# hila-chefer/Transformer-Explainability

Hardware: NVIDIA H100
Metric: explanations_per_sec (higher is better)
Workload: dtype f32

## Files before the change

transformer_explainability_b200/csrc/te_api.cu:

```cuda
#include <stdlib.h>
#include <string.h>
#include <atomic>
#include <string>

#include "../../include/te_b200.h"
#include "te_engine_util.h"
#include "te_kernels.h"
#include "te_rollout.h"
#include "te_zplus.h"
#include "te_gemm_tc.h"

static thread_local std::string g_last_error;
void te_set_last_error(const char* msg) { g_last_error = msg ? msg : ""; }

static std::atomic<long long> g_launches{0};
void te_count_launch() { g_launches.fetch_add(1, std::memory_order_relaxed); }
extern "C" long long te_kernel_launch_count(void) { return g_launches.load(); }

extern "C" const char* te_last_error(void) { return g_last_error.c_str(); }
extern "C" int te_version(void) { return 101; }

#define ST(s) reinterpret_cast<cudaStream_t>(s)
#define REQ(c, msg) do { if (!(c)) { te_set_last_error(msg); return TE_ERR_ARG; } } while (0)

// ... 214 lines not shown
void te_engine_set_cls_rows(int on) { g_cls_rows = on ? 1 : 0; }
static int g_gelu_split = -1;
bool te_engine_gelu_split() {
    if (g_gelu_split < 0) {
        const char* e = getenv("TE_B200_GELU_SPLIT");
        g_gelu_split = (e && e[0] == '0') ? 0 : 1;
    }
    return g_gelu_split != 0;
}
void te_engine_set_gelu_split(int on) { g_gelu_split = on ? 1 : 0; }

extern "C" int te_set_option(const char* name, int value) {
    REQ(name != nullptr, "te_set_option: null name");
    if (strcmp(name, "cls_row_top_block") == 0) { te_engine_set_cls_rows(value); return TE_OK; }
    if (strcmp(name, "gelu_split_fused") == 0) { te_engine_set_gelu_split(value); return TE_OK; }
    te_set_last_error("te_set_option: unknown option");
    return TE_ERR_ARG;
}

extern "C" int te_relevance_heatmap(const float* maps, int batch, int grid, int scale, float* out, void* stream) {
    REQ(maps && out && batch > 0 && grid > 0 && scale > 0, "te_relevance_heatmap: bad argument");
    return te_launch_relevance_heatmap(maps, out, batch, grid, scale, ST(stream));
}

extern "C" int te_head_reduce(const float* a, const float* g, const float* head_w, int batch, int heads, int n, int ld,
                              int mode, float* out, void* stream) {
    REQ(a && out && batch > 0 && heads > 0 && n > 0 && ld >= n && mode >= 0 && mode <= 2, "te_head_reduce: bad argument");
    return te_launch_head_reduce(a, g, head_w, out, batch, heads, n, ld, mode, ST(stream));
}
extern "C" int te_head_region_mean(const float* g, int batch, int heads, int n, int ld, int r0, int r1, int c0, int c1,
// ... 78 lines not shown
```

transformer_explainability_b200/csrc/te_gemm_tc.h:

```cpp
#pragma once
#include <cuda_bf16.h>
#include <type_traits>

#include "te_common.cuh"
#include "te_zplus.h"

bool te_tc_zplus_supported(long long rows, int in_features, int out_features, long long ldx);

template <class F>
struct TeDerived {
    template <class T> using P = std::conditional_t<std::is_const<F>::value, const T*, T*>;
    F *wp, *wn, *wpt, *wnt;
    F *wh, *wl, *wth, *wtl;
    F* wabs;
    P<__nv_bfloat16> bf_wpt, bf_wnt;
    F* gap;
    P<__nv_bfloat16> bf_wabs;
    P<__half> h_w, l_w;
    F* s_w;
    P<__half> h_wt;
    F* s_wt;
    P<__half> h_wpt, h_wnt;
    F *s_wpt, *s_wnt;
    static constexpr long long floats(int in_features, int out_features) { return 16LL * in_features * out_features; }
// ... 66 lines not shown
```

transformer_explainability_b200/csrc/te_tc_wgmma.cu:

```cuda
#include <cuda.h>
#include <cuda_bf16.h>
#include <cuda_fp16.h>
#include <cuda_runtime.h>
#include <string.h>
#include <algorithm>
#include <string>
#include <type_traits>
#include <utility>

#include "te_gemm_tc.h"
#include "te_wgmma.cuh"

namespace {

constexpr int BM = 128, NTHREADS = 256;

__device__ __forceinline__ uint32_t smem_u32(const void* p) { return (uint32_t)__cvta_generic_to_shared(p); }
__device__ __forceinline__ void fence_proxy_async() { asm volatile("fence.proxy.async.shared::cta;" ::: "memory"); }
__device__ __forceinline__ void wg_fence() { asm volatile("wgmma.fence.sync.aligned;" ::: "memory"); }
__device__ __forceinline__ void wg_commit() { asm volatile("wgmma.commit_group.sync.aligned;" ::: "memory"); }
__device__ __forceinline__ void wg_wait0() { asm volatile("wgmma.wait_group.sync.aligned 0;" ::: "memory"); }
__device__ __forceinline__ void wg_wait1() { asm volatile("wgmma.wait_group.sync.aligned 1;" ::: "memory"); }

__device__ __forceinline__ void mbar_init(uint32_t bar, uint32_t count) {
// ... 75 lines not shown
struct Stage {
    static constexpr int NTA = PRODS::NTA, NTB = PRODS::NTB;
    static constexpr int BYTES = NTA * TILE128 + NTB * BN * 128 + LAND;
    __host__ __device__ static constexpr uint32_t a(int i) { return (uint32_t)i * TILE128; }
    __host__ __device__ static constexpr uint32_t b(int j) { return (uint32_t)(NTA * TILE128 + j * BN * 128); }
    __host__ __device__ static constexpr uint32_t land() { return (uint32_t)(NTA * TILE128 + NTB * BN * 128); }
};

enum { OP_TF32 = 0, OP_BF16 = 1, OP_F16 = 2 };
template <int FMT, int NR>
__device__ __forceinline__ void wgmma_fmt(float (&d)[NR], uint64_t a, uint64_t b, uint32_t scale_d) {
    if constexpr (FMT == OP_TF32) wgmma_tf32(d, a, b, scale_d);
    else if constexpr (FMT == OP_BF16) wgmma_bf16(d, a, b, scale_d);
    else wgmma_f16(d, a, b, scale_d);
}
template <int FMT, class... T, size_t... I, int NA, int NR, int TA, int TB>
__device__ __forceinline__ void issue_kstep(Prods<T...>, std::index_sequence<I...>, float (&acc)[NA][NR], const uint64_t (&a)[TA],
                                            const uint64_t (&b)[TB], uint64_t q, uint32_t sd) {
    (wgmma_fmt<FMT>(acc[T::acc], a[T::a] + q, b[T::b] + q, Prods<T...>::first(I) ? sd : 1u), ...);
}
template <class P, int NA, int NR>
__device__ __forceinline__ void issue(uint32_t st, int wg, float (&acc)[NA][NR], uint32_t sd) {
    using L = typename P::L;
    uint64_t a[L::NTA], b[L::NTB];
#pragma unroll
    for (int i = 0; i < L::NTA; ++i) a[i] = sdesc(st + L::a(i) + (uint32_t)wg * 64u * 128u);
#pragma unroll
    for (int j = 0; j < L::NTB; ++j) b[j] = sdesc(st + L::b(j));
#pragma unroll
    for (int k = 0; k < 4; ++k)
        issue_kstep<P::FMT>(typename P::PRODS{}, std::make_index_sequence<P::PRODS::N>{}, acc, a, b, (uint64_t)(2 * k),
                            (k == 0) ? sd : 1u);
}

template <class F>
__device__ __forceinline__ void for_k32(int rows, const float* __restrict__ base, long long ld, long long row0, long long nrows,
                                        int k0, int K, int tid, F f) {
    for (int idx = tid; idx < rows * 8; idx += NTHREADS) {
        const int r = idx >> 3, c = idx & 7;
        const long long gr = row0 + r;
        const int k = k0 + 4 * c;
        float4 v = make_float4(0.f, 0.f, 0.f, 0.f);
        if (gr < nrows) {
            const float* src = base + gr * ld + k;
            if (k + 3 < K) v = *reinterpret_cast<const float4*>(src);
            else {
                if (k < K) v.x = src[0];
// ... 97 lines not shown
    const int tid = threadIdx.x, wg = tid >> 7;
    const int m0 = (col_fast ? blockIdx.y : blockIdx.x) * BM, n0 = (col_fast ? blockIdx.x : blockIdx.y) * P::BN;
    const int z = blockIdx.z;
    float acc[NA][NR];
    float tot[NT][NTR];
    zero(acc);
    zero(tot);

    const int kb = p.kblocks();
    p.load(smem, 0, m0, n0, z, tid);
    fence_proxy_async();
    __syncthreads();
    for (int it = 0; it < kb; ++it) {
        const bool fresh = P::CHUNK ? (it % P::CHUNK == 0) : (it == 0);
        wg_fence();
        issue<P>(smem_u32(smem + (it & 1) * STAGE), wg, acc, fresh ? 0u : 1u);
        wg_commit();
        if (it + 1 < kb) p.load(smem + ((it + 1) & 1) * STAGE, it + 1, m0, n0, z, tid);
        wg_wait0();
        if constexpr (P::CHUNK > 0)
            if ((it + 1) % P::CHUNK == 0 || it + 1 == kb) fold(p, acc, tot, m0, it / P::CHUNK, z, tid);
        fence_proxy_async();
        __syncthreads();
    }
    if constexpr (P::CHUNK > 0) p.epilogue(tot, m0, n0, z, tid, nullptr);
    else p.epilogue(acc, m0, n0, z, tid, nullptr);
}

template <class P>
__device__ __forceinline__ void tma_tiles(const P& p, const TmaArgs& ta, uint8_t* smem) {
    using L = typename P::L;
    constexpr int NR = P::BN / 2;
    constexpr int NA = P::PRODS::NACC;
    constexpr int STAGE = L::BYTES, EPI = epi_bytes<P>(), S = tma_stages(STAGE, EPI);
    constexpr int NT = P::CHUNK ? NA : 1, NTR = P::CHUNK ? NR : 1;
    static_assert(S >= 2, "a TMA problem needs two stages");
    __shared__ __align__(8) uint64_t bars[2 * S + 2];
    const int tid = threadIdx.x, wg = tid >> 7;
    const uint32_t full0 = smem_u32(bars), empty0 = full0 + 8u * S, st0 = smem_u32(smem);
    const uint32_t efull = full0 + 16u * S, eempty = efull + 8u, ebuf = st0 + (uint32_t)S * STAGE;
    if (tid == 0) {
        for (int s = 0; s < S; ++s) {
            mbar_init(full0 + 8u * s, 1);
            mbar_init(empty0 + 8u * s, 8);
        }
        mbar_init(efull, 1);
// ... 34 lines not shown
                                         m0, efull);
                        ephase ^= 1u;
                    }
                }
            }
        }
        return;
    }

    setmaxnreg_inc<232>();
    float acc[NA][NR];
    float tot[NT][NTR];
    auto release = [&](int s) {
        if ((tid & 31) == 0) mbar_arrive(empty0 + 8u * s);
    };
    auto consume = [&](uint32_t sd) {
        mbar_wait(full0 + 8u * stage, phase);
        if constexpr (P::FIX != FIX_NONE) {
            p.fix(smem + (uint32_t)stage * STAGE, wg, tid);
            fence_proxy_async();
            if constexpr (P::FIX == FIX_A) bar_named(1 + wg, 128);
            else bar_named(3, 256);
        }
        wg_fence();
        issue<P>(st0 + (uint32_t)stage * STAGE, wg, acc, sd);
        wg_commit();
    };
    auto next = [&] {
        if (++stage == S) { stage = 0; phase ^= 1u; }
    };
    constexpr int CH = P::CHUNK;
    uint32_t ephase = 0;
    for (int t = blockIdx.x; t < ntiles; t += gridDim.x) {
        int m0, n0, z;
        decode(t, m0, n0, z);
        zero(acc);
        zero(tot);
        for (int k0 = 0; k0 < kb; k0 += CH ? CH : kb) {
            const int k1 = CH ? min(k0 + CH, kb) : kb;
            consume(0u);
            for (int it = k0 + 1; it < k1; ++it) {
                const int prev = stage;
                next();
                consume(1u);
                wg_wait1();
                release(prev);
            }
            wg_wait0();
            release(stage);
            next();
            if constexpr (CH > 0) fold(p, acc, tot, m0, k0 / CH, z, tid);
        }
        if constexpr (EPI > 0) mbar_wait(efull, ephase);
        if constexpr (P::CHUNK > 0) p.epilogue(tot, m0, n0, z, tid, smem + (uint32_t)S * STAGE);
        else p.epilogue(acc, m0, n0, z, tid, smem + (uint32_t)S * STAGE);
        if constexpr (EPI > 0) {
            __syncwarp();
            if ((tid & 31) == 0) mbar_arrive(eempty);
            ephase ^= 1u;
        }
    }
}

template <class P>
__global__ void __launch_bounds__(P::TMA ? NTHREADS_TMA : NTHREADS, 1)
    wg_kernel(const P p, const __grid_constant__ TmaArgs ta, int col_fast) {
    extern __shared__ uint8_t smem_raw[];
    uint8_t* smem = smem_raw + ((1024u - (smem_u32(smem_raw) & 1023u)) & 1023u);
    if constexpr (P::TMA) tma_tiles(p, ta, smem);
    else reg_tile(p, smem, col_fast);
}

struct NoScale {
    __device__ __forceinline__ float chunk_scale(int, int, int) const { return 1.f; }
};

struct TmaTile {
    const void* base;
    long long rows, cols, ld;
    int box_rows;
    long long count = 0, cstride = 0;
};
template <class P>
__device__ __forceinline__ void produce_tiles(const TmaArgs& ta, uint32_t st, uint32_t bar, int it, int m0, int n0) {
// ... 256 lines not shown
    const void* b; const void* b_lo;
    const float* rs; const float* cs;
    LinOut o;
};
static_assert(sizeof(LinArgs) <= 128, "LinArgs: keep the kernel parameter within 128 bytes");
template <int EPI, int FORM>
struct LinProb : LinArgs {
    static constexpr bool F16 = FORM == LIN_F16X3 || FORM == LIN_F16, SPLIT = FORM == LIN_3XTF32 || FORM == LIN_F16X3;
    static constexpr int BN = FORM == LIN_TF32 && EPI == TE_TC_EPI_STORE ? 256 : 128;
    static constexpr int CHUNK = F16 ? 2 : SPLIT ? 4 : 0, FMT = F16 ? OP_F16 : OP_TF32;
    using PRODS = std::conditional_t<SPLIT, Split3, One>;
    using L = Stage<PRODS, BN>;
    static constexpr bool COL_FAST = true;
    static constexpr bool TMA = FORM != LIN_3XTF32;
    static constexpr int FIX = FORM == LIN_TF32 ? FIX_A : FIX_NONE;
    static constexpr int EPI_MAPS = TMA && EPI == TE_TC_EPI_GELU_BWD ? 1 : 0;
    __device__ int kblocks() const { return K / (F16 ? 64 : 32); }
    __device__ float chunk_scale(int row, int ch, int) const {
        if constexpr (F16) return row < o.M ? rs[(long long)row * rs_ld + ch] : 1.f;
        else return 1.f;
    }
    __device__ void fix(uint8_t* st, int wg, int tid) const {
        map_rows(st + L::a(0), 64 * wg, 64, tid & 127, 128, [](float4 v) { return tf32x4(v); });
    }
    TE_PRODUCE_TILES(LinProb)
    TmaTile tile(int i) const {
        if (i < L::NTA) return TmaTile{i == 0 ? a : a_lo, o.M, K, F16 ? K : lda, BM};
        if (i < NMAPS) return TmaTile{i == L::NTA ? b : b_lo, o.N, K, K, BN};
        return TmaTile{o.E, o.M, o.N, o.lde, BM};
    }
// ... 31 lines not shown
    }
    __device__ float2 efrag(const uint8_t* eb, int tid, int j, int row, int col) const {
        if constexpr (EPI_MAPS > 0) return epi_f2(eb, frag_row(tid, j), frag_col(tid, j));
        else return *reinterpret_cast<const float2*>(o.E + (long long)row * o.lde + col);
    }
};

enum { AT_STORE = 0, AT_MUL = 1, AT_SD = 2, AT_SOFTMAX = 3, AT_RESID = 4 };
template <int EPI, bool SP, int BN_>
struct NnProb : NoScale {
    static constexpr int BN = BN_, CHUNK = 0, FMT = OP_TF32;
    using PRODS = std::conditional_t<SP, One, Split3>;
    using L = Stage<PRODS, BN>;
    static constexpr bool TMA = true;
    static constexpr int FIX = FIX_AB, EPI_MAPS = 0;
    int N, H, dh, ld_out, batch;
    const float* a; long long lda; const float* b; long long ldb;
    const float* E; float* out; float alpha;
    __device__ int kblocks() const { return dh / 32; }
    static constexpr int NMAPS = 2;
    TmaTile tile(int i) const {
        return i == 0 ? TmaTile{a, (long long)batch * N, H * dh, lda, BM} : TmaTile{b, (long long)batch * N, H * dh, ldb, BN};
    }
    __device__ void produce(const TmaArgs& ta, uint32_t st, uint32_t bar, int kb, int m0, int n0, int bh) const {
        const int s = bh / H, k = (bh % H) * dh + kb * 32;
        mbar_expect_tx(bar, TILE128 + BN * 128);
        tma_load(st + L::a(0), &ta.map[0], k, s * N + m0, bar);
        tma_load(st + L::b(0), &ta.map[1], k, s * N + n0, bar);
    }
    __device__ void fix(uint8_t* st, int wg, int tid) const {
        fix_tf32<SP>(st + L::a(0), st + L::a(1), 64 * wg, 64, tid & 127, 128);
        fix_tf32<SP>(st + L::b(0), st + L::b(1), 0, BN, tid, 256);
    }
    __device__ void epilogue(float (&acc)[1][BN / 2], int m0, int n0, int bh, int tid, const uint8_t*) const {
        const int ncols = (N + 3) & ~3;
        if constexpr (EPI == AT_SOFTMAX) {
            float mx[2] = {-INFINITY, -INFINITY};
#pragma unroll
            for (int j = 0; j < BN / 2; ++j)
                if (n0 + frag_col(tid, j) < N) mx[(j >> 1) & 1] = fmaxf(mx[(j >> 1) & 1], alpha * acc[0][j]);
            float sum[2] = {0.f, 0.f}, m2[2];
#pragma unroll
            for (int h = 0; h < 2; ++h) {
                mx[h] = fmaxf(mx[h], __shfl_xor_sync(0xffffffffu, mx[h], 1));
                mx[h] = fmaxf(mx[h], __shfl_xor_sync(0xffffffffu, mx[h], 2));
                m2[h] = -mx[h] * 1.4426950408889634f;
            }
            const float a2 = alpha * 1.4426950408889634f;
// ... 40 lines not shown
            }
            *reinterpret_cast<float2*>(out + off) = make_float2(v[0], v[1]);
        }
        }
    }
};

template <int AMN, int EPI, bool SP, int BN_>
struct NkProb : NoScale {
    static constexpr int BN = BN_, CHUNK = SP ? 0 : 4, FMT = OP_TF32;
    using PRODS = std::conditional_t<SP, One, Split3>;
    static constexpr int LAND_A = AMN ? BM * 128 : 0, LAND_X = BN * 128;
    using L = Stage<PRODS, BN, LAND_A + LAND_X>;
    static constexpr bool TMA = true;
    static constexpr int FIX = FIX_AB, EPI_MAPS = 0;
    int N, H, NP, ld_out, n_out, n_pad, a_shared, batch;
    const float* map; const float* X; long long ldx;
    const float* rowscale; const float* E; float* out; float alpha;
    __device__ int kblocks() const { return (N + 31) / 32; }
    static constexpr int NMAPS = 2;
    TmaTile tile(int i) const {
        if (i == 0) return TmaTile{map, N, N, NP, AMN ? 32 : BM, (long long)batch * (a_shared ? 1 : H), (long long)N * NP};
        return TmaTile{X, N, n_pad, ldx, 32, batch, (long long)N * ldx};
    }
    __device__ void produce(const TmaArgs& ta, uint32_t st, uint32_t bar, int kb, int m0, int, int bh) const {
        const int s = bh / H, h = bh % H, za = a_shared ? s : bh;
        mbar_expect_tx(bar, (AMN ? LAND_A : TILE128) + LAND_X);
        if (AMN == 0) tma_load3(st + L::a(0), &ta.map[0], kb * 32, m0, za, bar);
#pragma unroll
        for (int j = 0; j < LAND_A / 4096; ++j) tma_load3(st + L::land() + j * 4096, &ta.map[0], m0 + 32 * j, kb * 32, za, bar);
#pragma unroll
        for (int j = 0; j < LAND_X / 4096; ++j)
            tma_load3(st + L::land() + LAND_A + j * 4096, &ta.map[1], h * BN + 32 * j, kb * 32, s, bar);
    }
    __device__ void fix(uint8_t* st, int wg, int tid) const {
        if (AMN) transpose_rows(st + L::land(), 64 * wg, 64, tid & 127, 128, put_tf32<SP>(st + L::a(0), st + L::a(1)));
        else fix_tf32<SP>(st + L::a(0), st + L::a(1), 64 * wg, 64, tid & 127, 128);
        transpose_rows(st + L::land() + LAND_A, 0, BN, tid, 256, put_tf32<SP>(st + L::b(0), st + L::b(1)));
    }
    __device__ void epilogue(float (&acc)[1][BN / 2], int m0, int, int bh, int tid, const uint8_t*) const {
        const int s = bh / H, h = bh % H;
        float2 ef[BN / 4];
#pragma unroll
        for (int j = 0; j < BN / 2; j += 2) {
            const int m = m0 + frag_row(tid, j), gcol = h * BN + frag_col(tid, j);
            ef[j / 2] = (EPI != AT_STORE && m < N && gcol < n_pad)
                            ? *reinterpret_cast<const float2*>(E + ((long long)s * N + m) * ld_out + gcol) : make_float2(0.f, 0.f);
        }
#pragma unroll
        for (int j = 0; j < BN / 2; j += 2) {
            const int m = m0 + frag_row(tid, j), gcol = h * BN + frag_col(tid, j);
            if (m >= N || gcol >= n_pad) continue;
// ... 39 lines not shown
    return fn;
}
bool encode_tile(CUtensorMap* map, const TmaTile& t, int esize) {
    const EncodeTiled fn = encode_tiled();
    const int rank = t.count > 0 ? 3 : 2;
    if (!fn || ((uintptr_t)t.base & 15u) || (t.ld * esize) % 16 != 0 || (t.cstride * esize) % 16 != 0 || t.rows < 1 || t.cols < 1)
        return false;
    const cuuint64_t dims[3] = {(cuuint64_t)t.cols, (cuuint64_t)t.rows, (cuuint64_t)t.count};
    const cuuint64_t strides[2] = {(cuuint64_t)(t.ld * esize), (cuuint64_t)(t.cstride * esize)};
    const cuuint32_t box[3] = {(cuuint32_t)(128 / esize), (cuuint32_t)t.box_rows, 1}, estr[3] = {1, 1, 1};
    return fn(map, esize == 4 ? CU_TENSOR_MAP_DATA_TYPE_FLOAT32 : CU_TENSOR_MAP_DATA_TYPE_UINT16, rank, const_cast<void*>(t.base),
              dims, strides, box, estr, CU_TENSOR_MAP_INTERLEAVE_NONE, CU_TENSOR_MAP_SWIZZLE_128B,
              CU_TENSOR_MAP_L2_PROMOTION_L2_256B, CU_TENSOR_MAP_FLOAT_OOB_FILL_NONE) == CUDA_SUCCESS;
}

template <class P>
int launch(const P& p, dim3 grid, cudaStream_t st) {
    TmaArgs ta;
    memset(&ta, 0, sizeof(ta));
    int col_fast = 0, threads = NTHREADS, smem = 2 * P::L::BYTES + 1024;
    if constexpr (P::TMA) {
        constexpr int ESIZE = P::FMT == OP_TF32 ? 4 : 2;
        static_assert(P::NMAPS + P::EPI_MAPS <= TMA_MAPS, "TmaArgs holds TMA_MAPS tensor maps");
        for (int i = 0; i < P::NMAPS + P::EPI_MAPS; ++i)
            if (!encode_tile(&ta.map[i], p.tile(i), i < P::NMAPS ? ESIZE : 4)) {
                te_set_last_error("te_tc: cannot encode a TMA tensor map (16-byte-aligned base and strides required)");
                return TE_ERR_ARG;
            }
        const long long tiles = (long long)grid.x * grid.y * grid.z;
        if (tiles > INT32_MAX) { te_set_last_error("te_tc: grid too large for one launch"); return TE_ERR_ARG; }
        ta.mtiles = (int)grid.x;
        ta.ntiles = (int)grid.y;
        ta.nz = (int)grid.z;
        grid = dim3((unsigned)std::min<long long>(tiles, sm_count()));
        threads = NTHREADS_TMA;
        smem = tma_stages(P::L::BYTES, epi_bytes<P>()) * P::L::BYTES + epi_bytes<P>() + 1024;
    } else {
        col_fast = P::COL_FAST && grid.x <= 65535;
        if (col_fast) grid = dim3(grid.y, grid.x, grid.z);
    }
    static unsigned long long done = 0;
    int dev = 0;
    if (cudaGetDevice(&dev) != cudaSuccess) { te_set_last_error("te_tc: cudaGetDevice failed"); return TE_ERR_CUDA; }
    if (!(done & (1ull << (dev & 63)))) {
        if (cudaFuncSetAttribute(wg_kernel<P>, cudaFuncAttributeMaxDynamicSharedMemorySize, smem) != cudaSuccess) {
            te_set_last_error("te_tc: cannot raise dynamic shared memory");
            return TE_ERR_CUDA;
        }
        done |= 1ull << (dev & 63);
    }
    if (grid.y > 65535 || grid.z > 65535) { te_set_last_error("te_tc: grid too large for one launch"); return TE_ERR_ARG; }
    wg_kernel<P><<<grid, threads, smem, st>>>(p, ta, col_fast);
    TE_CUDA_CHECK_LAUNCH();
    return TE_OK;
}
inline unsigned mtiles(long long M) { return (unsigned)((M + BM - 1) / BM); }

__global__ void prepare_weights_kernel(const float* __restrict__ w, float* __restrict__ d, int out_f, int in_f) {
    const TeDerived<float> dv(d, in_f, out_f);
    __shared__ float tile[32][33];
    const int bx = blockIdx.x * 32, by = blockIdx.y * 32;
    for (int i = threadIdx.y; i < 32; i += blockDim.y) {
        const int o = by + i, c = bx + threadIdx.x;
        float v = 0.f;
        if (o < out_f && c < in_f) {
            const long long idx = (long long)o * in_f + c;
            v = w[idx];
            dv.wp[idx] = to_tf32(fmaxf(v, 0.f));
            dv.wn[idx] = to_tf32(fminf(v, 0.f));
// ... 119 lines not shown
template <bool SINGLE, bool BF, int OUT>
int zs(const float* x, long long ldx, const void* xabs, const void* wa, const void* wb, const float* r, long long ldr,
       const float* y, long long ldy, const float* bias, void* out, float* hs, long long rows, int in_features, int out_features,
       cudaStream_t st, float s_scale, bool inh) {
    ZsProb<SINGLE, BF, OUT> p;
    p.M = (int)rows; p.N = out_features; p.K = in_features;
    p.x = x; p.ldx = ldx; p.xabs = xabs; p.wa = wa; p.wb = wb;
    p.r = r; p.ldr = ldr; p.y = y; p.ldy = ldy; p.bias = bias;
    p.out = out; p.ldo = out_features; p.hs = hs;
    p.sscale = s_scale; p.zsign = inh ? -1.f : 1.f;
    return launch(p, dim3(mtiles(p.M), p.N / 128), st);
}

}

long long te_tc_derived_floats(int in_features, int out_features) { return TeDerived<float>::floats(in_features, out_features); }

int te_tc_prepare_weights(const float* w, float* derived, int in_features, int out_features, cudaStream_t st) {
    dim3 grid((in_features + 31) / 32, (out_features + 31) / 32), block(32, 8);
    prepare_weights_kernel<<<grid, block, 0, st>>>(w, derived, out_features, in_features);
    TE_CUDA_CHECK_LAUNCH();
    const TeDerived<float> dv(derived, in_features, out_features);
    if (in_features % 8 == 0 && in_features >= 8 && a16(w))
        TE_TRY(te_tc_rowsplit_f16(w, in_features, out_features, in_features, dv.h_w, dv.l_w, dv.s_w, st));
    if (out_features % 8 == 0 && in_features >= 2) {
        TE_TRY(te_tc_rowsplit_f16(dv.wth, out_features, in_features, out_features, dv.h_wt, nullptr, dv.s_wt, st));
        TE_TRY(te_tc_rowsplit_f16(dv.wpt, out_features, in_features, out_features, dv.h_wpt, nullptr, dv.s_wpt, st));
        TE_TRY(te_tc_rowsplit_f16(dv.wnt, out_features, in_features, out_features, dv.h_wnt, nullptr, dv.s_wnt, st));
    }
    return TE_OK;
// ... 305 lines not shown
```

transformer_explainability_b200/csrc/te_wgmma.cuh:

```cuda
#pragma once
#include <stdint.h>

__device__ __forceinline__ void wgmma_tf32(float (&d)[32], uint64_t a, uint64_t b, uint32_t scale_d) {
    asm volatile(
        "{\n.reg .pred p;\nsetp.ne.b32 p, %34, 0;\n"
        "wgmma.mma_async.sync.aligned.m64n64k8.f32.tf32.tf32 {%0, %1, %2, %3, %4, %5, %6, %7, %8, %9, %10, %11, %12, %13, %14, %15, %16, %17, %18, %19, %20, %21, %22, %23, %24, %25, %26, %27, %28, %29, %30, %31}, %32, %33, p, 1, 1;\n}\n"
        : "+f"(d[0]), "+f"(d[1]), "+f"(d[2]), "+f"(d[3]), "+f"(d[4]), "+f"(d[5]), "+f"(d[6]), "+f"(d[7]), "+f"(d[8]), "+f"(d[9]), "+f"(d[10]), "+f"(d[11]), "+f"(d[12]), "+f"(d[13]), "+f"(d[14]), "+f"(d[15]), "+f"(d[16]), "+f"(d[17]), "+f"(d[18]), "+f"(d[19]), "+f"(d[20]), "+f"(d[21]), "+f"(d[22]), "+f"(d[23]), "+f"(d[24]), "+f"(d[25]), "+f"(d[26]), "+f"(d[27]), "+f"(d[28]), "+f"(d[29]), "+f"(d[30]), "+f"(d[31])
        : "l"(a), "l"(b), "r"(scale_d));
}
__device__ __forceinline__ void wgmma_tf32(float (&d)[64], uint64_t a, uint64_t b, uint32_t scale_d) {
    asm volatile(
        "{\n.reg .pred p;\nsetp.ne.b32 p, %66, 0;\n"
        "wgmma.mma_async.sync.aligned.m64n128k8.f32.tf32.tf32 {%0, %1, %2, %3, %4, %5, %6, %7, %8, %9, %10, %11, %12, %13, %14, %15, %16, %17, %18, %19, %20, %21, %22, %23, %24, %25, %26, %27, %28, %29, %30, %31, %32, %33, %34, %35, %36, %37, %38, %39, %40, %41, %42, %43, %44, %45, %46, %47, %48, %49, %50, %51, %52, %53, %54, %55, %56, %57, %58, %59, %60, %61, %62, %63}, %64, %65, p, 1, 1;\n}\n"
        : "+f"(d[0]), "+f"(d[1]), "+f"(d[2]), "+f"(d[3]), "+f"(d[4]), "+f"(d[5]), "+f"(d[6]), "+f"(d[7]), "+f"(d[8]), "+f"(d[9]), "+f"(d[10]), "+f"(d[11]), "+f"(d[12]), "+f"(d[13]), "+f"(d[14]), "+f"(d[15]), "+f"(d[16]), "+f"(d[17]), "+f"(d[18]), "+f"(d[19]), "+f"(d[20]), "+f"(d[21]), "+f"(d[22]), "+f"(d[23]), "+f"(d[24]), "+f"(d[25]), "+f"(d[26]), "+f"(d[27]), "+f"(d[28]), "+f"(d[29]), "+f"(d[30]), "+f"(d[31]), "+f"(d[32]), "+f"(d[33]), "+f"(d[34]), "+f"(d[35]), "+f"(d[36]), "+f"(d[37]), "+f"(d[38]), "+f"(d[39]), "+f"(d[40]), "+f"(d[41]), "+f"(d[42]), "+f"(d[43]), "+f"(d[44]), "+f"(d[45]), "+f"(d[46]), "+f"(d[47]), "+f"(d[48]), "+f"(d[49]), "+f"(d[50]), "+f"(d[51]), "+f"(d[52]), "+f"(d[53]), "+f"(d[54]), "+f"(d[55]), "+f"(d[56]), "+f"(d[57]), "+f"(d[58]), "+f"(d[59]), "+f"(d[60]), "+f"(d[61]), "+f"(d[62]), "+f"(d[63])
        : "l"(a), "l"(b), "r"(scale_d));
}
__device__ __forceinline__ void wgmma_tf32(float (&d)[128], uint64_t a, uint64_t b, uint32_t scale_d) {
    asm volatile(
        "{\n.reg .pred p;\nsetp.ne.b32 p, %130, 0;\n"
        "wgmma.mma_async.sync.aligned.m64n256k8.f32.tf32.tf32 {%0, %1, %2, %3, %4, %5, %6, %7, %8, %9, %10, %11, %12, %13, %14, %15, %16, %17, %18, %19, %20, %21, %22, %23, %24, %25, %26, %27, %28, %29, %30, %31, %32, %33, %34, %35, %36, %37, %38, %39, %40, %41, %42, %43, %44, %45, %46, %47, %48, %49, %50, %51, %52, %53, %54, %55, %56, %57, %58, %59, %60, %61, %62, %63, %64, %65, %66, %67, %68, %69, %70, %71, %72, %73, %74, %75, %76, %77, %78, %79, %80, %81, %82, %83, %84, %85, %86, %87, %88, %89, %90, %91, %92, %93, %94, %95, %96, %97, %98, %99, %100, %101, %102, %103, %104, %105, %106, %107, %108, %109, %110, %111, %112, %113, %114, %115, %116, %117, %118, %119, %120, %121, %122, %123, %124, %125, %126, %127}, %128, %129, p, 1, 1;\n}\n"
        : "+f"(d[0]), "+f"(d[1]), "+f"(d[2]), "+f"(d[3]), "+f"(d[4]), "+f"(d[5]), "+f"(d[6]), "+f"(d[7]), "+f"(d[8]), "+f"(d[9]), "+f"(d[10]), "+f"(d[11]), "+f"(d[12]), "+f"(d[13]), "+f"(d[14]), "+f"(d[15]), "+f"(d[16]), "+f"(d[17]), "+f"(d[18]), "+f"(d[19]), "+f"(d[20]), "+f"(d[21]), "+f"(d[22]), "+f"(d[23]), "+f"(d[24]), "+f"(d[25]), "+f"(d[26]), "+f"(d[27]), "+f"(d[28]), "+f"(d[29]), "+f"(d[30]), "+f"(d[31]), "+f"(d[32]), "+f"(d[33]), "+f"(d[34]), "+f"(d[35]), "+f"(d[36]), "+f"(d[37]), "+f"(d[38]), "+f"(d[39]), "+f"(d[40]), "+f"(d[41]), "+f"(d[42]), "+f"(d[43]), "+f"(d[44]), "+f"(d[45]), "+f"(d[46]), "+f"(d[47]), "+f"(d[48]), "+f"(d[49]), "+f"(d[50]), "+f"(d[51]), "+f"(d[52]), "+f"(d[53]), "+f"(d[54]), "+f"(d[55]), "+f"(d[56]), "+f"(d[57]), "+f"(d[58]), "+f"(d[59]), "+f"(d[60]), "+f"(d[61]), "+f"(d[62]), "+f"(d[63]), "+f"(d[64]), "+f"(d[65]), "+f"(d[66]), "+f"(d[67]), "+f"(d[68]), "+f"(d[69]), "+f"(d[70]), "+f"(d[71]), "+f"(d[72]), "+f"(d[73]), "+f"(d[74]), "+f"(d[75]), "+f"(d[76]), "+f"(d[77]), "+f"(d[78]), "+f"(d[79]), "+f"(d[80]), "+f"(d[81]), "+f"(d[82]), "+f"(d[83]), "+f"(d[84]), "+f"(d[85]), "+f"(d[86]), "+f"(d[87]), "+f"(d[88]), "+f"(d[89]), "+f"(d[90]), "+f"(d[91]), "+f"(d[92]), "+f"(d[93]), "+f"(d[94]), "+f"(d[95]), "+f"(d[96]), "+f"(d[97]), "+f"(d[98]), "+f"(d[99]), "+f"(d[100]), "+f"(d[101]), "+f"(d[102]), "+f"(d[103]), "+f"(d[104]), "+f"(d[105]), "+f"(d[106]), "+f"(d[107]), "+f"(d[108]), "+f"(d[109]), "+f"(d[110]), "+f"(d[111]), "+f"(d[112]), "+f"(d[113]), "+f"(d[114]), "+f"(d[115]), "+f"(d[116]), "+f"(d[117]), "+f"(d[118]), "+f"(d[119]), "+f"(d[120]), "+f"(d[121]), "+f"(d[122]), "+f"(d[123]), "+f"(d[124]), "+f"(d[125]), "+f"(d[126]), "+f"(d[127])
        : "l"(a), "l"(b), "r"(scale_d));
}
__device__ __forceinline__ void wgmma_f16(float (&d)[32], uint64_t a, uint64_t b, uint32_t scale_d) {
// ... 12 lines not shown
}
__device__ __forceinline__ void wgmma_bf16(float (&d)[32], uint64_t a, uint64_t b, uint32_t scale_d) {
    asm volatile(
        "{\n.reg .pred p;\nsetp.ne.b32 p, %34, 0;\n"
        "wgmma.mma_async.sync.aligned.m64n64k16.f32.bf16.bf16 {%0, %1, %2, %3, %4, %5, %6, %7, %8, %9, %10, %11, %12, %13, %14, %15, %16, %17, %18, %19, %20, %21, %22, %23, %24, %25, %26, %27, %28, %29, %30, %31}, %32, %33, p, 1, 1, 0, 0;\n}\n"
        : "+f"(d[0]), "+f"(d[1]), "+f"(d[2]), "+f"(d[3]), "+f"(d[4]), "+f"(d[5]), "+f"(d[6]), "+f"(d[7]), "+f"(d[8]), "+f"(d[9]), "+f"(d[10]), "+f"(d[11]), "+f"(d[12]), "+f"(d[13]), "+f"(d[14]), "+f"(d[15]), "+f"(d[16]), "+f"(d[17]), "+f"(d[18]), "+f"(d[19]), "+f"(d[20]), "+f"(d[21]), "+f"(d[22]), "+f"(d[23]), "+f"(d[24]), "+f"(d[25]), "+f"(d[26]), "+f"(d[27]), "+f"(d[28]), "+f"(d[29]), "+f"(d[30]), "+f"(d[31])
        : "l"(a), "l"(b), "r"(scale_d));
}
__device__ __forceinline__ void wgmma_bf16(float (&d)[64], uint64_t a, uint64_t b, uint32_t scale_d) {
    asm volatile(
        "{\n.reg .pred p;\nsetp.ne.b32 p, %66, 0;\n"
        "wgmma.mma_async.sync.aligned.m64n128k16.f32.bf16.bf16 {%0, %1, %2, %3, %4, %5, %6, %7, %8, %9, %10, %11, %12, %13, %14, %15, %16, %17, %18, %19, %20, %21, %22, %23, %24, %25, %26, %27, %28, %29, %30, %31, %32, %33, %34, %35, %36, %37, %38, %39, %40, %41, %42, %43, %44, %45, %46, %47, %48, %49, %50, %51, %52, %53, %54, %55, %56, %57, %58, %59, %60, %61, %62, %63}, %64, %65, p, 1, 1, 0, 0;\n}\n"
        : "+f"(d[0]), "+f"(d[1]), "+f"(d[2]), "+f"(d[3]), "+f"(d[4]), "+f"(d[5]), "+f"(d[6]), "+f"(d[7]), "+f"(d[8]), "+f"(d[9]), "+f"(d[10]), "+f"(d[11]), "+f"(d[12]), "+f"(d[13]), "+f"(d[14]), "+f"(d[15]), "+f"(d[16]), "+f"(d[17]), "+f"(d[18]), "+f"(d[19]), "+f"(d[20]), "+f"(d[21]), "+f"(d[22]), "+f"(d[23]), "+f"(d[24]), "+f"(d[25]), "+f"(d[26]), "+f"(d[27]), "+f"(d[28]), "+f"(d[29]), "+f"(d[30]), "+f"(d[31]), "+f"(d[32]), "+f"(d[33]), "+f"(d[34]), "+f"(d[35]), "+f"(d[36]), "+f"(d[37]), "+f"(d[38]), "+f"(d[39]), "+f"(d[40]), "+f"(d[41]), "+f"(d[42]), "+f"(d[43]), "+f"(d[44]), "+f"(d[45]), "+f"(d[46]), "+f"(d[47]), "+f"(d[48]), "+f"(d[49]), "+f"(d[50]), "+f"(d[51]), "+f"(d[52]), "+f"(d[53]), "+f"(d[54]), "+f"(d[55]), "+f"(d[56]), "+f"(d[57]), "+f"(d[58]), "+f"(d[59]), "+f"(d[60]), "+f"(d[61]), "+f"(d[62]), "+f"(d[63])
        : "l"(a), "l"(b), "r"(scale_d));
}
```

Measured before the change: 918.9.

## Feed TF32 wgmma A operand from registers instead of shared-memory fix pass

For TF32 GEMM problems that previously rewrote the A tile in shared memory (rounding to TF32) before issuing wgmma, the A fragments are now loaded straight into registers, rounded there, and passed to a register-A wgmma variant. The consumer loop ping-pongs between two fragment buffers so the next fragment can load while the previous wgmma is in flight. This removes the shared-memory write-back, proxy fence and per-warpgroup barrier for A. In exchange it adds register pressure and per-thread shared-memory reads. The path is enabled by default and can be turned off with a runtime option.

```diff
diff --git a/transformer_explainability_b200/csrc/te_api.cu b/transformer_explainability_b200/csrc/te_api.cu
--- a/transformer_explainability_b200/csrc/te_api.cu
+++ b/transformer_explainability_b200/csrc/te_api.cu
@@ -252,6 +252,7 @@
     REQ(name != nullptr, "te_set_option: null name");
     if (strcmp(name, "cls_row_top_block") == 0) { te_engine_set_cls_rows(value); return TE_OK; }
     if (strcmp(name, "gelu_split_fused") == 0) { te_engine_set_gelu_split(value); return TE_OK; }
+    if (strcmp(name, "a_from_registers") == 0) { te_tc_set_a_from_registers(value); return TE_OK; }
     te_set_last_error("te_set_option: unknown option");
     return TE_ERR_ARG;
 }
diff --git a/transformer_explainability_b200/csrc/te_gemm_tc.h b/transformer_explainability_b200/csrc/te_gemm_tc.h
--- a/transformer_explainability_b200/csrc/te_gemm_tc.h
+++ b/transformer_explainability_b200/csrc/te_gemm_tc.h
@@ -4,6 +4,8 @@
 
 #include "te_common.cuh"
 #include "te_zplus.h"
+
+void te_tc_set_a_from_registers(int on);
 
 bool te_tc_zplus_supported(long long rows, int in_features, int out_features, long long ldx);
 
diff --git a/transformer_explainability_b200/csrc/te_tc_wgmma.cu b/transformer_explainability_b200/csrc/te_tc_wgmma.cu
--- a/transformer_explainability_b200/csrc/te_tc_wgmma.cu
+++ b/transformer_explainability_b200/csrc/te_tc_wgmma.cu
@@ -113,13 +113,24 @@
     else if constexpr (FMT == OP_BF16) wgmma_bf16(d, a, b, scale_d);
     else wgmma_f16(d, a, b, scale_d);
 }
-template <int FMT, class... T, size_t... I, int NA, int NR, int TA, int TB>
+template <int FMT, int NR>
+__device__ __forceinline__ void wgmma_fmt(float (&d)[NR], const uint32_t (&a)[4], uint64_t b, uint32_t scale_d) {
+    static_assert(FMT == OP_TF32, "A from registers: TF32 only");
+    wgmma_tf32(d, a, b, scale_d);
+}
+template <int FMT, bool AR, class T, int NA, int NR, int TA, int TB>
+__device__ __forceinline__ void issue_prod(float (&acc)[NA][NR], const uint64_t (&a)[TA], const uint64_t (&b)[TB],
+                                           const uint32_t (&fr)[4], uint64_t q, uint32_t sd) {
+    if constexpr (AR && T::a == 0) wgmma_fmt<FMT>(acc[T::acc], fr, b[T::b] + q, sd);
+    else wgmma_fmt<FMT>(acc[T::acc], a[T::a] + q, b[T::b] + q, sd);
+}
+template <int FMT, bool AR, class... T, size_t... I, int NA, int NR, int TA, int TB>
 __device__ __forceinline__ void issue_kstep(Prods<T...>, std::index_sequence<I...>, float (&acc)[NA][NR], const uint64_t (&a)[TA],
-                                            const uint64_t (&b)[TB], uint64_t q, uint32_t sd) {
-    (wgmma_fmt<FMT>(acc[T::acc], a[T::a] + q, b[T::b] + q, Prods<T...>::first(I) ? sd : 1u), ...);
-}
-template <class P, int NA, int NR>
-__device__ __forceinline__ void issue(uint32_t st, int wg, float (&acc)[NA][NR], uint32_t sd) {
+                                            const uint64_t (&b)[TB], const uint32_t (&fr)[4], uint64_t q, uint32_t sd) {
+    (issue_prod<FMT, AR, T>(acc, a, b, fr, q, Prods<T...>::first(I) ? sd : 1u), ...);
+}
+template <class P, bool AR, int NA, int NR>
+__device__ __forceinline__ void issue(uint32_t st, int wg, float (&acc)[NA][NR], uint32_t sd, const uint32_t (&fr)[4][4]) {
     using L = typename P::L;
     uint64_t a[L::NTA], b[L::NTB];
 #pragma unroll
@@ -128,8 +139,28 @@
     for (int j = 0; j < L::NTB; ++j) b[j] = sdesc(st + L::b(j));
 #pragma unroll
     for (int k = 0; k < 4; ++k)
-        issue_kstep<P::FMT>(typename P::PRODS{}, std::make_index_sequence<P::PRODS::N>{}, acc, a, b, (uint64_t)(2 * k),
-                            (k == 0) ? sd : 1u);
+        issue_kstep<P::FMT, AR>(typename P::PRODS{}, std::make_index_sequence<P::PRODS::N>{}, acc, a, b, fr[k], (uint64_t)(2 * k),
+                                (k == 0) ? sd : 1u);
+}
+
+template <class P, class = void>
+struct ARegs : std::false_type {};
+template <class P>
+struct ARegs<P, std::void_t<decltype(P::A_REGS)>> : std::bool_constant<P::A_REGS> {};
+int g_a_regs = 1;
+
+template <class P>
+__device__ __forceinline__ void a_frag(const uint8_t* tile, int tid, uint32_t (&fr)[4][4]) {
+    const int lane = tid & 31, r = 64 * (tid >> 7) + 16 * ((tid >> 5) & 3), g = lane >> 2;
+    const uint8_t* row = tile + (r + g) * 128 + (lane & 3) * 4;
+#pragma unroll
+    for (int k = 0; k < 4; ++k)
+#pragma unroll
+        for (int h = 0; h < 2; ++h) {
+            const uint8_t* e = row + (((2 * k + h) ^ g) << 4);
+            fr[k][2 * h] = P::areg(*reinterpret_cast<const uint32_t*>(e));
+            fr[k][2 * h + 1] = P::areg(*reinterpret_cast<const uint32_t*>(e + 8 * 128));
+        }
 }
 
 template <class F>
@@ -257,7 +288,8 @@
     for (int it = 0; it < kb; ++it) {
         const bool fresh = P::CHUNK ? (it % P::CHUNK == 0) : (it == 0);
         wg_fence();
-        issue<P>(smem_u32(smem + (it & 1) * STAGE), wg, acc, fresh ? 0u : 1u);
+        const uint32_t no_frag[4][4] = {};
+        issue<P, false>(smem_u32(smem + (it & 1) * STAGE), wg, acc, fresh ? 0u : 1u, no_frag);
         wg_commit();
         if (it + 1 < kb) p.load(smem + ((it + 1) & 1) * STAGE, it + 1, m0, n0, z, tid);
         wg_wait0();
@@ -270,9 +302,10 @@
     else p.epilogue(acc, m0, n0, z, tid, nullptr);
 }
 
-template <class P>
+template <class P, bool AR>
 __device__ __forceinline__ void tma_tiles(const P& p, const TmaArgs& ta, uint8_t* smem) {
     using L = typename P::L;
+    static_assert(!AR || ARegs<P>::value, "A from registers: an A_REGS problem");
     constexpr int NR = P::BN / 2;
     constexpr int NA = P::PRODS::NACC;
     constexpr int STAGE = L::BYTES, EPI = epi_bytes<P>(), S = tma_stages(STAGE, EPI);
@@ -337,21 +370,36 @@
     auto release = [&](int s) {
         if ((tid & 31) == 0) mbar_arrive(empty0 + 8u * s);
     };
-    auto consume = [&](uint32_t sd) {
+    auto consume = [&](uint32_t sd, uint32_t (&fr)[4][4]) {
         mbar_wait(full0 + 8u * stage, phase);
-        if constexpr (P::FIX != FIX_NONE) {
+        if constexpr (AR) {
+            a_frag<P>(smem + (uint32_t)stage * STAGE + L::a(0), tid, fr);
+            if constexpr (P::FIX == FIX_AB) {
+                p.fix_b(smem + (uint32_t)stage * STAGE, tid);
+                fence_proxy_async();
+                bar_named(3, 256);
+            }
+        } else if constexpr (P::FIX != FIX_NONE) {
             p.fix(smem + (uint32_t)stage * STAGE, wg, tid);
             fence_proxy_async();
             if constexpr (P::FIX == FIX_A) bar_named(1 + wg, 128);
             else bar_named(3, 256);
         }
         wg_fence();
-        issue<P>(st0 + (uint32_t)stage * STAGE, wg, acc, sd);
+        issue<P, AR>(st0 + (uint32_t)stage * STAGE, wg, acc, sd, fr);
         wg_commit();
     };
     auto next = [&] {
         if (++stage == S) { stage = 0; phase ^= 1u; }
     };
+    auto step = [&](uint32_t (&fr)[4][4]) {
+        const int prev = stage;
+        next();
+        consume(1u, fr);
+        wg_wait1();
+        release(prev);
+    };
+    uint32_t fa[4][4], fb[4][4];
     constexpr int CH = P::CHUNK;
     uint32_t ephase = 0;
     for (int t = blockIdx.x; t < ntiles; t += gridDim.x) {
@@ -361,13 +409,16 @@
         zero(tot);
         for (int k0 = 0; k0 < kb; k0 += CH ? CH : kb) {
             const int k1 = CH ? min(k0 + CH, kb) : kb;
-            consume(0u);
-            for (int it = k0 + 1; it < k1; ++it) {
-                const int prev = stage;
-                next();
-                consume(1u);
-                wg_wait1();
-                release(prev);
+            consume(0u, fa);
+            if constexpr (AR) {
+                int it = k0 + 1;
+                for (; it + 1 < k1; it += 2) {
+                    step(fb);
+                    step(fa);
+                }
+                if (it < k1) step(fb);
+            } else {
+                for (int it = k0 + 1; it < k1; ++it) step(fa);
             }
             wg_wait0();
             release(stage);
@@ -385,12 +436,12 @@
     }
 }
 
-template <class P>
+template <class P, bool AR>
 __global__ void __launch_bounds__(P::TMA ? NTHREADS_TMA : NTHREADS, 1)
     wg_kernel(const P p, const __grid_constant__ TmaArgs ta, int col_fast) {
     extern __shared__ uint8_t smem_raw[];
     uint8_t* smem = smem_raw + ((1024u - (smem_u32(smem_raw) & 1023u)) & 1023u);
-    if constexpr (P::TMA) tma_tiles(p, ta, smem);
+    if constexpr (P::TMA) tma_tiles<P, AR>(p, ta, smem);
     else reg_tile(p, smem, col_fast);
 }
 
@@ -677,6 +728,8 @@
     static constexpr bool COL_FAST = true;
     static constexpr bool TMA = FORM != LIN_3XTF32;
     static constexpr int FIX = FORM == LIN_TF32 ? FIX_A : FIX_NONE;
+    static constexpr bool A_REGS = FORM == LIN_TF32;
+    __device__ static uint32_t areg(uint32_t v) { return __float_as_uint(to_tf32(__uint_as_float(v))); }
     static constexpr int EPI_MAPS = TMA && EPI == TE_TC_EPI_GELU_BWD ? 1 : 0;
     __device__ int kblocks() const { return K / (F16 ? 64 : 32); }
     __device__ float chunk_scale(int row, int ch, int) const {
@@ -738,6 +791,8 @@
     using L = Stage<PRODS, BN>;
     static constexpr bool TMA = true;
     static constexpr int FIX = FIX_AB, EPI_MAPS = 0;
+    static constexpr bool A_REGS = SP;
+    __device__ static uint32_t areg(uint32_t v) { return __float_as_uint(to_tf32(__uint_as_float(v))); }
     int N, H, dh, ld_out, batch;
     const float* a; long long lda; const float* b; long long ldb;
     const float* E; float* out; float alpha;
@@ -754,8 +809,9 @@
     }
     __device__ void fix(uint8_t* st, int wg, int tid) const {
         fix_tf32<SP>(st + L::a(0), st + L::a(1), 64 * wg, 64, tid & 127, 128);
-        fix_tf32<SP>(st + L::b(0), st + L::b(1), 0, BN, tid, 256);
-    }
+        fix_b(st, tid);
+    }
+    __device__ void fix_b(uint8_t* st, int tid) const { fix_tf32<SP>(st + L::b(0), st + L::b(1), 0, BN, tid, 256); }
     __device__ void epilogue(float (&acc)[1][BN / 2], int m0, int n0, int bh, int tid, const uint8_t*) const {
         const int ncols = (N + 3) & ~3;
         if constexpr (EPI == AT_SOFTMAX) {
@@ -826,6 +882,8 @@
     using L = Stage<PRODS, BN, LAND_A + LAND_X>;
     static constexpr bool TMA = true;
     static constexpr int FIX = FIX_AB, EPI_MAPS = 0;
+    static constexpr bool A_REGS = SP && AMN == 0;
+    __device__ static uint32_t areg(uint32_t v) { return __float_as_uint(to_tf32(__uint_as_float(v))); }
     int N, H, NP, ld_out, n_out, n_pad, a_shared, batch;
     const float* map; const float* X; long long ldx;
     const float* rowscale; const float* E; float* out; float alpha;
@@ -848,6 +906,9 @@
     __device__ void fix(uint8_t* st, int wg, int tid) const {
         if (AMN) transpose_rows(st + L::land(), 64 * wg, 64, tid & 127, 128, put_tf32<SP>(st + L::a(0), st + L::a(1)));
         else fix_tf32<SP>(st + L::a(0), st + L::a(1), 64 * wg, 64, tid & 127, 128);
+        fix_b(st, tid);
+    }
+    __device__ void fix_b(uint8_t* st, int tid) const {
         transpose_rows(st + L::land() + LAND_A, 0, BN, tid, 256, put_tf32<SP>(st + L::b(0), st + L::b(1)));
     }
     __device__ void epilogue(float (&acc)[1][BN / 2], int m0, int, int bh, int tid, const uint8_t*) const {
@@ -917,6 +978,22 @@
               CU_TENSOR_MAP_L2_PROMOTION_L2_256B, CU_TENSOR_MAP_FLOAT_OOB_FILL_NONE) == CUDA_SUCCESS;
 }
 
+template <class P, bool AR>
+int launch_kernel(const P& p, const TmaArgs& ta, dim3 grid, int threads, int smem, int col_fast, cudaStream_t st) {
+    static unsigned long long done = 0;
+    int dev = 0;
+    if (cudaGetDevice(&dev) != cudaSuccess) { te_set_last_error("te_tc: cudaGetDevice failed"); return TE_ERR_CUDA; }
+    if (!(done & (1ull << (dev & 63)))) {
+        if (cudaFuncSetAttribute(wg_kernel<P, AR>, cudaFuncAttributeMaxDynamicSharedMemorySize, smem) != cudaSuccess) {
+            te_set_last_error("te_tc: cannot raise dynamic shared memory");
+            return TE_ERR_CUDA;
+        }
+        done |= 1ull << (dev & 63);
+    }
+    wg_kernel<P, AR><<<grid, threads, smem, st>>>(p, ta, col_fast);
+    TE_CUDA_CHECK_LAUNCH();
+    return TE_OK;
+}
 template <class P>
 int launch(const P& p, dim3 grid, cudaStream_t st) {
     TmaArgs ta;
@@ -942,20 +1019,10 @@
         col_fast = P::COL_FAST && grid.x <= 65535;
         if (col_fast) grid = dim3(grid.y, grid.x, grid.z);
     }
-    static unsigned long long done = 0;
-    int dev = 0;
-    if (cudaGetDevice(&dev) != cudaSuccess) { te_set_last_error("te_tc: cudaGetDevice failed"); return TE_ERR_CUDA; }
-    if (!(done & (1ull << (dev & 63)))) {
-        if (cudaFuncSetAttribute(wg_kernel<P>, cudaFuncAttributeMaxDynamicSharedMemorySize, smem) != cudaSuccess) {
-            te_set_last_error("te_tc: cannot raise dynamic shared memory");
-            return TE_ERR_CUDA;
-        }
-        done |= 1ull << (dev & 63);
-    }
     if (grid.y > 65535 || grid.z > 65535) { te_set_last_error("te_tc: grid too large for one launch"); return TE_ERR_ARG; }
-    wg_kernel<P><<<grid, threads, smem, st>>>(p, ta, col_fast);
-    TE_CUDA_CHECK_LAUNCH();
-    return TE_OK;
+    if constexpr (ARegs<P>::value)
+        if (g_a_regs) return launch_kernel<P, true>(p, ta, grid, threads, smem, col_fast, st);
+    return launch_kernel<P, false>(p, ta, grid, threads, smem, col_fast, st);
 }
 inline unsigned mtiles(long long M) { return (unsigned)((M + BM - 1) / BM); }
 
@@ -1105,6 +1172,8 @@
 
 }
 
+void te_tc_set_a_from_registers(int on) { g_a_regs = on ? 1 : 0; }
+
 long long te_tc_derived_floats(int in_features, int out_features) { return TeDerived<float>::floats(in_features, out_features); }
 
 int te_tc_prepare_weights(const float* w, float* derived, int in_features, int out_features, cudaStream_t st) {
diff --git a/transformer_explainability_b200/csrc/te_wgmma.cuh b/transformer_explainability_b200/csrc/te_wgmma.cuh
--- a/transformer_explainability_b200/csrc/te_wgmma.cuh
+++ b/transformer_explainability_b200/csrc/te_wgmma.cuh
@@ -50,3 +50,24 @@
         : "+f"(d[0]), "+f"(d[1]), "+f"(d[2]), "+f"(d[3]), "+f"(d[4]), "+f"(d[5]), "+f"(d[6]), "+f"(d[7]), "+f"(d[8]), "+f"(d[9]), "+f"(d[10]), "+f"(d[11]), "+f"(d[12]), "+f"(d[13]), "+f"(d[14]), "+f"(d[15]), "+f"(d[16]), "+f"(d[17]), "+f"(d[18]), "+f"(d[19]), "+f"(d[20]), "+f"(d[21]), "+f"(d[22]), "+f"(d[23]), "+f"(d[24]), "+f"(d[25]), "+f"(d[26]), "+f"(d[27]), "+f"(d[28]), "+f"(d[29]), "+f"(d[30]), "+f"(d[31]), "+f"(d[32]), "+f"(d[33]), "+f"(d[34]), "+f"(d[35]), "+f"(d[36]), "+f"(d[37]), "+f"(d[38]), "+f"(d[39]), "+f"(d[40]), "+f"(d[41]), "+f"(d[42]), "+f"(d[43]), "+f"(d[44]), "+f"(d[45]), "+f"(d[46]), "+f"(d[47]), "+f"(d[48]), "+f"(d[49]), "+f"(d[50]), "+f"(d[51]), "+f"(d[52]), "+f"(d[53]), "+f"(d[54]), "+f"(d[55]), "+f"(d[56]), "+f"(d[57]), "+f"(d[58]), "+f"(d[59]), "+f"(d[60]), "+f"(d[61]), "+f"(d[62]), "+f"(d[63])
         : "l"(a), "l"(b), "r"(scale_d));
 }
+__device__ __forceinline__ void wgmma_tf32(float (&d)[32], const uint32_t (&a)[4], uint64_t b, uint32_t scale_d) {
+    asm volatile(
+        "{\n.reg .pred p;\nsetp.ne.b32 p, %37, 0;\n"
+        "wgmma.mma_async.sync.aligned.m64n64k8.f32.tf32.tf32 {%0, %1, %2, %3, %4, %5, %6, %7, %8, %9, %10, %11, %12, %13, %14, %15, %16, %17, %18, %19, %20, %21, %22, %23, %24, %25, %26, %27, %28, %29, %30, %31}, {%32, %33, %34, %35}, %36, p, 1, 1;\n}\n"
+        : "+f"(d[0]), "+f"(d[1]), "+f"(d[2]), "+f"(d[3]), "+f"(d[4]), "+f"(d[5]), "+f"(d[6]), "+f"(d[7]), "+f"(d[8]), "+f"(d[9]), "+f"(d[10]), "+f"(d[11]), "+f"(d[12]), "+f"(d[13]), "+f"(d[14]), "+f"(d[15]), "+f"(d[16]), "+f"(d[17]), "+f"(d[18]), "+f"(d[19]), "+f"(d[20]), "+f"(d[21]), "+f"(d[22]), "+f"(d[23]), "+f"(d[24]), "+f"(d[25]), "+f"(d[26]), "+f"(d[27]), "+f"(d[28]), "+f"(d[29]), "+f"(d[30]), "+f"(d[31])
+        : "r"(a[0]), "r"(a[1]), "r"(a[2]), "r"(a[3]), "l"(b), "r"(scale_d));
+}
+__device__ __forceinline__ void wgmma_tf32(float (&d)[64], const uint32_t (&a)[4], uint64_t b, uint32_t scale_d) {
+    asm volatile(
+        "{\n.reg .pred p;\nsetp.ne.b32 p, %69, 0;\n"
+        "wgmma.mma_async.sync.aligned.m64n128k8.f32.tf32.tf32 {%0, %1, %2, %3, %4, %5, %6, %7, %8, %9, %10, %11, %12, %13, %14, %15, %16, %17, %18, %19, %20, %21, %22, %23, %24, %25, %26, %27, %28, %29, %30, %31, %32, %33, %34, %35, %36, %37, %38, %39, %40, %41, %42, %43, %44, %45, %46, %47, %48, %49, %50, %51, %52, %53, %54, %55, %56, %57, %58, %59, %60, %61, %62, %63}, {%64, %65, %66, %67}, %68, p, 1, 1;\n}\n"
+        : "+f"(d[0]), "+f"(d[1]), "+f"(d[2]), "+f"(d[3]), "+f"(d[4]), "+f"(d[5]), "+f"(d[6]), "+f"(d[7]), "+f"(d[8]), "+f"(d[9]), "+f"(d[10]), "+f"(d[11]), "+f"(d[12]), "+f"(d[13]), "+f"(d[14]), "+f"(d[15]), "+f"(d[16]), "+f"(d[17]), "+f"(d[18]), "+f"(d[19]), "+f"(d[20]), "+f"(d[21]), "+f"(d[22]), "+f"(d[23]), "+f"(d[24]), "+f"(d[25]), "+f"(d[26]), "+f"(d[27]), "+f"(d[28]), "+f"(d[29]), "+f"(d[30]), "+f"(d[31]), "+f"(d[32]), "+f"(d[33]), "+f"(d[34]), "+f"(d[35]), "+f"(d[36]), "+f"(d[37]), "+f"(d[38]), "+f"(d[39]), "+f"(d[40]), "+f"(d[41]), "+f"(d[42]), "+f"(d[43]), "+f"(d[44]), "+f"(d[45]), "+f"(d[46]), "+f"(d[47]), "+f"(d[48]), "+f"(d[49]), "+f"(d[50]), "+f"(d[51]), "+f"(d[52]), "+f"(d[53]), "+f"(d[54]), "+f"(d[55]), "+f"(d[56]), "+f"(d[57]), "+f"(d[58]), "+f"(d[59]), "+f"(d[60]), "+f"(d[61]), "+f"(d[62]), "+f"(d[63])
+        : "r"(a[0]), "r"(a[1]), "r"(a[2]), "r"(a[3]), "l"(b), "r"(scale_d));
+}
+__device__ __forceinline__ void wgmma_tf32(float (&d)[128], const uint32_t (&a)[4], uint64_t b, uint32_t scale_d) {
+    asm volatile(
+        "{\n.reg .pred p;\nsetp.ne.b32 p, %133, 0;\n"
+        "wgmma.mma_async.sync.aligned.m64n256k8.f32.tf32.tf32 {%0, %1, %2, %3, %4, %5, %6, %7, %8, %9, %10, %11, %12, %13, %14, %15, %16, %17, %18, %19, %20, %21, %22, %23, %24, %25, %26, %27, %28, %29, %30, %31, %32, %33, %34, %35, %36, %37, %38, %39, %40, %41, %42, %43, %44, %45, %46, %47, %48, %49, %50, %51, %52, %53, %54, %55, %56, %57, %58, %59, %60, %61, %62, %63, %64, %65, %66, %67, %68, %69, %70, %71, %72, %73, %74, %75, %76, %77, %78, %79, %80, %81, %82, %83, %84, %85, %86, %87, %88, %89, %90, %91, %92, %93, %94, %95, %96, %97, %98, %99, %100, %101, %102, %103, %104, %105, %106, %107, %108, %109, %110, %111, %112, %113, %114, %115, %116, %117, %118, %119, %120, %121, %122, %123, %124, %125, %126, %127}, {%128, %129, %130, %131}, %132, p, 1, 1;\n}\n"
+        : "+f"(d[0]), "+f"(d[1]), "+f"(d[2]), "+f"(d[3]), "+f"(d[4]), "+f"(d[5]), "+f"(d[6]), "+f"(d[7]), "+f"(d[8]), "+f"(d[9]), "+f"(d[10]), "+f"(d[11]), "+f"(d[12]), "+f"(d[13]), "+f"(d[14]), "+f"(d[15]), "+f"(d[16]), "+f"(d[17]), "+f"(d[18]), "+f"(d[19]), "+f"(d[20]), "+f"(d[21]), "+f"(d[22]), "+f"(d[23]), "+f"(d[24]), "+f"(d[25]), "+f"(d[26]), "+f"(d[27]), "+f"(d[28]), "+f"(d[29]), "+f"(d[30]), "+f"(d[31]), "+f"(d[32]), "+f"(d[33]), "+f"(d[34]), "+f"(d[35]), "+f"(d[36]), "+f"(d[37]), "+f"(d[38]), "+f"(d[39]), "+f"(d[40]), "+f"(d[41]), "+f"(d[42]), "+f"(d[43]), "+f"(d[44]), "+f"(d[45]), "+f"(d[46]), "+f"(d[47]), "+f"(d[48]), "+f"(d[49]), "+f"(d[50]), "+f"(d[51]), "+f"(d[52]), "+f"(d[53]), "+f"(d[54]), "+f"(d[55]), "+f"(d[56]), "+f"(d[57]), "+f"(d[58]), "+f"(d[59]), "+f"(d[60]), "+f"(d[61]), "+f"(d[62]), "+f"(d[63]), "+f"(d[64]), "+f"(d[65]), "+f"(d[66]), "+f"(d[67]), "+f"(d[68]), "+f"(d[69]), "+f"(d[70]), "+f"(d[71]), "+f"(d[72]), "+f"(d[73]), "+f"(d[74]), "+f"(d[75]), "+f"(d[76]), "+f"(d[77]), "+f"(d[78]), "+f"(d[79]), "+f"(d[80]), "+f"(d[81]), "+f"(d[82]), "+f"(d[83]), "+f"(d[84]), "+f"(d[85]), "+f"(d[86]), "+f"(d[87]), "+f"(d[88]), "+f"(d[89]), "+f"(d[90]), "+f"(d[91]), "+f"(d[92]), "+f"(d[93]), "+f"(d[94]), "+f"(d[95]), "+f"(d[96]), "+f"(d[97]), "+f"(d[98]), "+f"(d[99]), "+f"(d[100]), "+f"(d[101]), "+f"(d[102]), "+f"(d[103]), "+f"(d[104]), "+f"(d[105]), "+f"(d[106]), "+f"(d[107]), "+f"(d[108]), "+f"(d[109]), "+f"(d[110]), "+f"(d[111]), "+f"(d[112]), "+f"(d[113]), "+f"(d[114]), "+f"(d[115]), "+f"(d[116]), "+f"(d[117]), "+f"(d[118]), "+f"(d[119]), "+f"(d[120]), "+f"(d[121]), "+f"(d[122]), "+f"(d[123]), "+f"(d[124]), "+f"(d[125]), "+f"(d[126]), "+f"(d[127])
+        : "r"(a[0]), "r"(a[1]), "r"(a[2]), "r"(a[3]), "l"(b), "r"(scale_d));
+}
```

Result: faster. 929.5, median of 6 (+1.1%).
